# bitsauce/Carla-ppo

Measured on NVIDIA H100. Metric: VAE frames/sec @ batch 4096, higher is better.
Workload: dtype f32

## Files before the change

carla_ppo_b200/csrc/tapgemm.cuh:

```cuda
#pragma once
#include "common.cuh"

namespace cpb {

constexpr int kMaxTaps = 25;

struct Tap {
    int dy, dx;
    long long src_off;
    long long w_off;
};

struct TapClass {
    int ntaps;
    int py, px;
    int Ho, Wo;
    Tap taps[kMaxTaps];
};

struct TapGemmParams {
    const float* src;
    const float* wmat;
    const float* bias;
    const float* mask;
    float* dst;
    int batch;
    int Hs, Ws;
    int src_pitch;
    long long src_img;
    int sstride;
    int C;
    int N;
    int ldw;
    int Hd, Wd;
    int dstride;
    int dst_pitch;
    long long dst_img;
    int relu;
    int check;
    int nclass;
    int ybatch;
    long long w_ystride, bias_ystride, dst_ystride;
    int ksplit;
    float* kpartial;
    long long kpartial_stride;
    const float* wk_hi;
    const float* wk_lo;
    int quad;
    int quad_cb;
    int quad_lcb;
    int cluster;
    int debug;
    int passes;
    TapClass cls[4];
};

int32_t launch_tapgemm(const TapGemmParams& p, cudaStream_t stream);
constexpr int kMaxKSplit = 8;
int tapgemm_pick_ksplit(int rows, int N, int ybatch, int K);
int32_t launch_ksplit_reduce(const TapGemmParams& p, cudaStream_t stream);
int32_t tapgemm_init();

struct TcWeightJob {
    long long src_off;
    long long dst_hi, dst_lo;
    int mode;
    int k, cb, cs;
    int N, C;
    long long count;
    int round_nearest;
};
__host__ __device__ constexpr int tc_bn(int N) { return N % 64 == 0 ? 64 : 32; }
constexpr int kMaxTcWeightJobs = 12;
struct TcWeightTable {
    int njobs;
    long long total;
    TcWeightJob jobs[kMaxTcWeightJobs];
};
int32_t tc_tapgemm_init();
int tc_tapgemm_pick_ksplit(int K);
bool tc_tapgemm_supported(const TapGemmParams& p);
int32_t launch_tc_tapgemm(const TapGemmParams& p, cudaStream_t stream);
int32_t launch_tc_weights(const float* params, float* dst, const TcWeightTable& table, cudaStream_t stream);

}
```

carla_ppo_b200/csrc/tc_common.cuh:

```cuda
#pragma once
#include "common.cuh"

namespace cpb {
namespace tc {

constexpr int TBM = 128;
constexpr int TBK = 32;
constexpr int A_TILE_BYTES = TBM * TBK * 4;
constexpr int kMaxBN = 64;

__device__ __forceinline__ uint32_t smem_u32(const void* p) { return (uint32_t)__cvta_generic_to_shared(p); }

__host__ __device__ __forceinline__ uint32_t row_magic(int d) { return (uint32_t)((0x80000000ull + (uint32_t)d - 1) / (uint32_t)d); }
__device__ __forceinline__ int row_of(int rem, uint32_t magic) { return (int)__umulhi((uint32_t)rem << 1, magic); }

__device__ __forceinline__ void mbar_init(uint64_t* bar, uint32_t count) {
    asm volatile("mbarrier.init.shared::cta.b64 [%0], %1;" ::"r"(smem_u32(bar)), "r"(count));
}
__device__ __forceinline__ void mbar_wait(uint64_t* bar, uint32_t parity) {
    const uint32_t addr = smem_u32(bar);
    uint32_t ok = 0;
    for (uint32_t spin = 0; !ok; ++spin) {
        asm volatile(
            "{\n\t.reg .pred p;\n\t"
            "mbarrier.try_wait.parity.shared::cta.b64 p, [%1], %2;\n\t"
            "selp.u32 %0, 1, 0, p;\n\t}"
            : "=r"(ok)
            : "r"(addr), "r"(parity)
            : "memory");
        if (spin > (1u << 28)) __trap();
    }
}
__device__ __forceinline__ void mbar_arrive(uint64_t* bar) {
    asm volatile("{\n\t.reg .b64 st;\n\tmbarrier.arrive.shared::cta.b64 st, [%0];\n\t}" ::"r"(smem_u32(bar)) : "memory");
}
__device__ __forceinline__ void mbar_arrive_cluster(uint64_t* bar, uint32_t rank) {
    asm volatile(
        "{\n\t.reg .b32 ra;\n\t"
        "mapa.shared::cluster.u32 ra, %0, %1;\n\t"
        "mbarrier.arrive.release.cluster.shared::cluster.b64 _, [ra];\n\t}"
        ::"r"(smem_u32(bar)), "r"(rank) : "memory");
}
__device__ __forceinline__ void fence_async_smem() { asm volatile("fence.proxy.async.shared::cta;" ::: "memory"); }

__device__ __forceinline__ uint64_t make_desc(uint32_t smem_addr) {
    uint64_t d = 0;
    d |= (uint64_t)((smem_addr >> 4) & 0x3FFF);
    d |= (uint64_t)1 << 16;
    d |= (uint64_t)(1024 >> 4) << 32;
    d |= (uint64_t)1 << 62;
    return d;
}

__device__ __forceinline__ void wgmma_fence() { asm volatile("wgmma.fence.sync.aligned;" ::: "memory"); }
__device__ __forceinline__ void wgmma_commit() { asm volatile("wgmma.commit_group.sync.aligned;" ::: "memory"); }
template <int N>
__device__ __forceinline__ void wgmma_wait() { asm volatile("wgmma.wait_group.sync.aligned %0;" ::"n"(N) : "memory"); }
template <int R>
__device__ __forceinline__ void fence_regs(float* d) {
#pragma unroll
    for (int i = 0; i < R; ++i) asm volatile("" : "+f"(d[i])::"memory");
}

template <int N>
__device__ __forceinline__ void wgmma_tf32(float* d, uint64_t adesc, uint64_t bdesc, uint32_t scale_d);
template <>
__device__ __forceinline__ void wgmma_tf32<32>(float* d, uint64_t adesc, uint64_t bdesc, uint32_t scale_d) {
    asm volatile(
        "{\n\t.reg .pred p;\n\t"
        "setp.ne.b32 p, %18, 0;\n\t"
        "wgmma.mma_async.sync.aligned.m64n32k8.f32.tf32.tf32 {%0,%1,%2,%3,%4,%5,%6,%7,%8,%9,%10,%11,%12,%13,%14,%15}, %16, %17, p, 1, 1;\n\t}"
        : "+f"(d[0]), "+f"(d[1]), "+f"(d[2]), "+f"(d[3]), "+f"(d[4]), "+f"(d[5]), "+f"(d[6]), "+f"(d[7]), "+f"(d[8]), "+f"(d[9]), "+f"(d[10]), "+f"(d[11]), "+f"(d[12]), "+f"(d[13]), "+f"(d[14]), "+f"(d[15])
        : "l"(adesc), "l"(bdesc), "r"(scale_d));
}

template <>
__device__ __forceinline__ void wgmma_tf32<64>(float* d, uint64_t adesc, uint64_t bdesc, uint32_t scale_d) {
    asm volatile(
        "{\n\t.reg .pred p;\n\t"
        "setp.ne.b32 p, %34, 0;\n\t"
        "wgmma.mma_async.sync.aligned.m64n64k8.f32.tf32.tf32 {%0,%1,%2,%3,%4,%5,%6,%7,%8,%9,%10,%11,%12,%13,%14,%15,%16,%17,%18,%19,%20,%21,%22,%23,%24,%25,%26,%27,%28,%29,%30,%31}, %32, %33, p, 1, 1;\n\t}"
        : "+f"(d[0]), "+f"(d[1]), "+f"(d[2]), "+f"(d[3]), "+f"(d[4]), "+f"(d[5]), "+f"(d[6]), "+f"(d[7]), "+f"(d[8]), "+f"(d[9]), "+f"(d[10]), "+f"(d[11]), "+f"(d[12]), "+f"(d[13]), "+f"(d[14]), "+f"(d[15]), "+f"(d[16]), "+f"(d[17]), "+f"(d[18]), "+f"(d[19]), "+f"(d[20]), "+f"(d[21]), "+f"(d[22]), "+f"(d[23]), "+f"(d[24]), "+f"(d[25]), "+f"(d[26]), "+f"(d[27]), "+f"(d[28]), "+f"(d[29]), "+f"(d[30]), "+f"(d[31])
        : "l"(adesc), "l"(bdesc), "r"(scale_d));
}

template <int N>
__device__ __forceinline__ void wgmma_tf32_rs(float* d, const uint32_t* a, uint64_t bdesc, uint32_t scale_d);
template <>
__device__ __forceinline__ void wgmma_tf32_rs<32>(float* d, const uint32_t* a, uint64_t bdesc, uint32_t scale_d) {
    asm volatile(
        "{\n\t.reg .pred p;\n\t"
        "setp.ne.b32 p, %21, 0;\n\t"
        "wgmma.mma_async.sync.aligned.m64n32k8.f32.tf32.tf32 {%0,%1,%2,%3,%4,%5,%6,%7,%8,%9,%10,%11,%12,%13,%14,%15}, {%16,%17,%18,%19}, %20, p, 1, 1;\n\t}"
        : "+f"(d[0]), "+f"(d[1]), "+f"(d[2]), "+f"(d[3]), "+f"(d[4]), "+f"(d[5]), "+f"(d[6]), "+f"(d[7]), "+f"(d[8]), "+f"(d[9]), "+f"(d[10]), "+f"(d[11]), "+f"(d[12]), "+f"(d[13]), "+f"(d[14]), "+f"(d[15])
        : "r"(a[0]), "r"(a[1]), "r"(a[2]), "r"(a[3]), "l"(bdesc), "r"(scale_d));
}

template <>
__device__ __forceinline__ void wgmma_tf32_rs<64>(float* d, const uint32_t* a, uint64_t bdesc, uint32_t scale_d) {
    asm volatile(
        "{\n\t.reg .pred p;\n\t"
        "setp.ne.b32 p, %37, 0;\n\t"
        "wgmma.mma_async.sync.aligned.m64n64k8.f32.tf32.tf32 {%0,%1,%2,%3,%4,%5,%6,%7,%8,%9,%10,%11,%12,%13,%14,%15,%16,%17,%18,%19,%20,%21,%22,%23,%24,%25,%26,%27,%28,%29,%30,%31}, {%32,%33,%34,%35}, %36, p, 1, 1;\n\t}"
        : "+f"(d[0]), "+f"(d[1]), "+f"(d[2]), "+f"(d[3]), "+f"(d[4]), "+f"(d[5]), "+f"(d[6]), "+f"(d[7]), "+f"(d[8]), "+f"(d[9]), "+f"(d[10]), "+f"(d[11]), "+f"(d[12]), "+f"(d[13]), "+f"(d[14]), "+f"(d[15]), "+f"(d[16]), "+f"(d[17]), "+f"(d[18]), "+f"(d[19]), "+f"(d[20]), "+f"(d[21]), "+f"(d[22]), "+f"(d[23]), "+f"(d[24]), "+f"(d[25]), "+f"(d[26]), "+f"(d[27]), "+f"(d[28]), "+f"(d[29]), "+f"(d[30]), "+f"(d[31])
        : "r"(a[0]), "r"(a[1]), "r"(a[2]), "r"(a[3]), "l"(bdesc), "r"(scale_d));
}

__device__ __forceinline__ void split_tf32(float x, float& hi, float& lo) {
    hi = __uint_as_float(__float_as_uint(x) & 0xffffe000u);
    lo = x - hi;
}

__device__ __forceinline__ uint32_t round_tf32(float x) {
    uint32_t r;
    asm("cvt.rna.tf32.f32 %0, %1;" : "=r"(r) : "f"(x));
    return r;
}

}
}
```

carla_ppo_b200/csrc/tc_tapgemm.cu:

```cuda
#include "tapgemm.cuh"
#include "tc_common.cuh"

namespace cpb {

namespace {

using namespace tc;

template <int BN, int PASSES>
struct TcCfg {
    static constexpr int B_TILE_BYTES = BN * TBK * 4;
    static constexpr int B_IMAGES = PASSES == 3 ? 2 : 1;
    static constexpr int STAGE_BYTES = A_TILE_BYTES + B_IMAGES * B_TILE_BYTES;
    static constexpr int OUT_BYTES = TBM * BN * 4;
    static constexpr int STAGES = (224 * 1024 - OUT_BYTES) / STAGE_BYTES;
    static constexpr int SMEM_BYTES = STAGES * STAGE_BYTES + OUT_BYTES + 1024;
};
constexpr int CHUNK_KB = 4;

constexpr int kConsumerWarps = 8;
constexpr int kLoaderWarp0 = 8;
constexpr int kLoaderWarps = 4;
constexpr int kLoaderThreads = kLoaderWarps * 32;
constexpr int kEpilogueWarp0 = 12;
constexpr int kEpilogueWarps = 4;
constexpr int kEpilogueThreads = kEpilogueWarps * 32;
constexpr int kTcThreads = 512;
constexpr int kLaunchRegs = 128, kConsumerRegs = 168, kSideRegs = 80;
template <int R> __device__ __forceinline__ void reg_grow() { asm volatile("setmaxnreg.inc.sync.aligned.u32 %0;" ::"n"(R)); }
template <int R> __device__ __forceinline__ void reg_shrink() { asm volatile("setmaxnreg.dec.sync.aligned.u32 %0;" ::"n"(R)); }

int g_tc_cluster = 1;
int g_tc_clusters[2][2] = {{0, 0}, {0, 0}};

__device__ __forceinline__ uint32_t cluster_ctarank() { uint32_t r; asm volatile("mov.u32 %0, %%cluster_ctarank;" : "=r"(r)); return r; }
__device__ __forceinline__ uint32_t cluster_id_x() { uint32_t r; asm volatile("mov.u32 %0, %%clusterid.x;" : "=r"(r)); return r; }
__device__ __forceinline__ uint32_t cluster_count_x() { uint32_t r; asm volatile("mov.u32 %0, %%nclusterid.x;" : "=r"(r)); return r; }
__device__ __forceinline__ void cluster_sync_all() {
    asm volatile("barrier.cluster.arrive.release.aligned;" ::: "memory");
    asm volatile("barrier.cluster.wait.acquire.aligned;" ::: "memory");
}
__device__ __forceinline__ void mbar_expect_tx(uint64_t* bar, uint32_t bytes) {
    asm volatile("{\n\t.reg .b64 st;\n\tmbarrier.arrive.expect_tx.shared::cta.b64 st, [%0], %1;\n\t}" ::"r"(smem_u32(bar)), "r"(bytes) : "memory");
}
__device__ __forceinline__ void bulk_g2s(uint32_t dst, const void* src, uint32_t bytes, uint64_t* bar, uint16_t mask, bool multicast) {
    if (multicast)
        asm volatile("cp.async.bulk.shared::cluster.global.mbarrier::complete_tx::bytes.multicast::cluster [%0], [%1], %2, [%3], %4;"
                     ::"r"(dst), "l"(src), "r"(bytes), "r"(smem_u32(bar)), "h"(mask) : "memory");
    else
        asm volatile("cp.async.bulk.shared::cluster.global.mbarrier::complete_tx::bytes [%0], [%1], %2, [%3];"
                     ::"r"(dst), "l"(src), "r"(bytes), "r"(smem_u32(bar)) : "memory");
}

template <int BN, int PASSES, bool KSPLIT>
__global__ void __maxnreg__(kLaunchRegs)
tc_tapgemm_kernel(const __grid_constant__ TapGemmParams p, const int mgroups, const int total_w) {
    static_assert(PASSES == 3 || PASSES == 1, "3xTF32 or a single TF32 pass");
    using Cfg = TcCfg<BN, PASSES>;
    constexpr int STAGES = Cfg::STAGES;
    constexpr int B_TILE_BYTES = Cfg::B_TILE_BYTES;
    constexpr int STAGE_BYTES = Cfg::STAGE_BYTES;

    extern __shared__ uint8_t smem_raw[];
    __shared__ uint64_t full_bar[STAGES];
    __shared__ uint64_t empty_bar[STAGES];
    __shared__ uint64_t out_full;
    __shared__ uint64_t out_empty;

    const int tid = threadIdx.x;
    const int warp = __shfl_sync(0xffffffffu, tid >> 5, 0), lane = tid & 31;
    const int ntn = p.N / BN;
    const int CS = (int)p.cluster;
    const int rank = CS > 1 ? (int)cluster_ctarank() : 0;
    const int cl_id = CS > 1 ? (int)cluster_id_x() : (int)blockIdx.x;
    const int cl_n = CS > 1 ? (int)cluster_count_x() : (int)gridDim.x;
    const uint16_t cl_mask = (uint16_t)((1u << CS) - 1u);
    const uint32_t smem_base = (smem_u32(smem_raw) + 1023u) & ~1023u;
    const uint32_t out_base = smem_base + STAGES * STAGE_BYTES;

    if (tid == 0) {
#pragma unroll
        for (int s = 0; s < STAGES; ++s) { mbar_init(&full_bar[s], kLoaderThreads + 1); mbar_init(&empty_bar[s], (uint32_t)(kConsumerWarps * CS)); }
        mbar_init(&out_full, kConsumerWarps);
        mbar_init(&out_empty, kEpilogueWarps);
        asm volatile("fence.mbarrier_init.release.cluster;" ::: "memory");
    }
    __syncthreads();
    if (CS > 1) cluster_sync_all();

    auto st_z = [&](int st) { return st / (ntn * mgroups); };
    auto st_y = [&](int st) { return st % ntn; };
    auto st_m0 = [&](int st) { return (long long)(((st / ntn) % mgroups) * CS + rank) * TBM; };
    const int kb_per_tap = p.C / TBK;
    const int ksplit = KSPLIT ? p.ksplit : 1;
    auto split_kb = [&](int nkb, int ks) { return (int)((long long)nkb * ks / ksplit); };

    if (warp >= kEpilogueWarp0) {
        reg_shrink<kSideRegs>();
        constexpr int CPR = BN / 4;
        constexpr int RPP = kEpilogueThreads / CPR;
        constexpr int NR = TBM / RPP;
        constexpr uint32_t SKIP = 0xffffffffu;
        const int et = tid - kEpilogueWarp0 * 32;
        const int ec = et % CPR, er = et / CPR;
        const uint32_t o_src = out_base + (uint32_t)(er * (BN * 4) + ((ec ^ ((er & 3) << 1)) << 4));
        uint32_t phO = 0;
        for (int w = cl_id; w < total_w && !(p.debug & 16); w += cl_n) {
            const int st = KSPLIT ? w / ksplit : w, ks = KSPLIT ? w - st * ksplit : 0;
            const TapClass& cls = p.cls[st_z(st)];
            float* const dst = KSPLIT ? p.dst + (long long)ks * p.kpartial_stride : p.dst;
            const int Wo = cls.Wo, HoWo = cls.Ho * Wo;
            const uint32_t M = (uint32_t)p.batch * (uint32_t)HoWo;
            const uint32_t wo_magic = row_magic(Wo);
            const int col = st_y(st) * BN + ec * 4;
            int ch = col, qy = 0, qx = 0;
            if (p.quad) {
                const int c = col >> p.quad_lcb;
                ch = col & (p.quad_cb - 1);
                qy = c >> 1; qx = c & 1;
            }
            const uint32_t m0 = (uint32_t)st_m0(st) + (uint32_t)er;
            const int n0 = (int)(m0 / (uint32_t)HoWo);
            const int rem0 = (int)(m0 - (uint32_t)n0 * (uint32_t)HoWo);
            uint32_t m = m0;
            int n = n0, rem = rem0;
            auto next_off = [&]() {
                const int oy = row_of(rem, wo_magic);
                const int ox = rem - oy * Wo;
                const uint32_t img = (uint32_t)n * (uint32_t)p.dst_img;
                bool ok = m < M;
                uint32_t off;
                if (p.quad) {
                    const int y = oy * 2 + qy, x = ox * 2 + qx;
                    ok = ok && y < p.Hd && x < p.Wd;
                    off = img + (uint32_t)((y * p.Wd + x) * p.dst_pitch + ch);
                } else {
                    off = img + (uint32_t)(((oy * p.dstride + cls.py) * p.Wd + (ox * p.dstride + cls.px)) * p.dst_pitch + col);
                }
                m += RPP; rem += RPP;
                while (rem >= HoWo) { rem -= HoWo; ++n; }
                return ok ? off : SKIP;
            };
            uint32_t keep[NR / 8];
            if (p.mask) {
#pragma unroll 1
                for (int b = 0; b < NR / 8; ++b) {
                    uint32_t offs[8];
                    float4 mk[8];
#pragma unroll
                    for (int u = 0; u < 8; ++u) offs[u] = next_off();
#pragma unroll
                    for (int u = 0; u < 8; ++u)
                        mk[u] = offs[u] != SKIP ? __ldg(reinterpret_cast<const float4*>(p.mask + offs[u])) : make_float4(0.f, 0.f, 0.f, 0.f);
                    uint32_t bits = 0u;
#pragma unroll
                    for (int u = 0; u < 8; ++u)
                        bits |= ((mk[u].x > 0.f ? 1u : 0u) | (mk[u].y > 0.f ? 2u : 0u) | (mk[u].z > 0.f ? 4u : 0u) | (mk[u].w > 0.f ? 8u : 0u)) << (4 * u);
#pragma unroll
                    for (int q = 0; q < NR / 8 - 1; ++q) keep[q] = keep[q + 1];
                    keep[NR / 8 - 1] = bits;
                }
                m = m0; n = n0; rem = rem0;
            }
            float4 bias = make_float4(0.f, 0.f, 0.f, 0.f);
            if (p.bias) bias = __ldg(reinterpret_cast<const float4*>(p.bias + ch));

            mbar_wait(&out_full, phO);
            phO ^= 1u;
#pragma unroll 1
            for (int b = 0; b < NR / 8; ++b) {
                uint32_t offs[8];
                float4 sums[8];
#pragma unroll
                for (int u = 0; u < 8; ++u)
                    asm volatile("ld.shared.v4.f32 {%0, %1, %2, %3}, [%4];" : "=f"(sums[u].x), "=f"(sums[u].y), "=f"(sums[u].z), "=f"(sums[u].w)
                                 : "r"(o_src + (uint32_t)((8 * b + u) * RPP * BN * 4)));
#pragma unroll
                for (int u = 0; u < 8; ++u) offs[u] = next_off();
                const uint32_t bits = p.mask ? keep[0] : 0u;
#pragma unroll
                for (int q = 0; q < NR / 8 - 1; ++q) keep[q] = keep[q + 1];
#pragma unroll
                for (int u = 0; u < 8; ++u) {
                    if (offs[u] == SKIP) continue;
                    float4 o = sums[u];
                    if (p.bias) { o.x += bias.x; o.y += bias.y; o.z += bias.z; o.w += bias.w; }
                    if (p.relu) { o.x = fmaxf(o.x, 0.f); o.y = fmaxf(o.y, 0.f); o.z = fmaxf(o.z, 0.f); o.w = fmaxf(o.w, 0.f); }
                    if (p.mask) {
                        const uint32_t k = bits >> (4 * u);
                        o.x = (k & 1u) ? o.x : 0.f; o.y = (k & 2u) ? o.y : 0.f; o.z = (k & 4u) ? o.z : 0.f; o.w = (k & 8u) ? o.w : 0.f;
                    }
                    *reinterpret_cast<float4*>(dst + offs[u]) = o;
                }
            }
            __syncwarp();
            if (lane == 0) mbar_arrive(&out_empty);
        }
    } else if (warp >= kLoaderWarp0) {
        reg_shrink<kSideRegs>();
        const int tl = tid - kLoaderWarp0 * 32;
        const int a_chunk = tl & 7;
        const uint32_t a_soff0 = (uint32_t)((tl >> 6) * 1024 + ((tl >> 3) & 7) * 128 + ((a_chunk ^ ((tl >> 3) & 7)) << 4));
        constexpr int RPP = kLoaderThreads / 8;
        constexpr int RPT = TBM / RPP;

        int wA = cl_id, stA = 0, tapA = 0, cA = 0;
        int kbLeftA = 0;
        int ntapsA = 0;
        int offA = 0;
        uint32_t tapbitA = 1u;
        const TapClass* clsA = &p.cls[0];
        uint32_t a_base[RPT];
        uint32_t a_taps[RPT];
        auto setup_rows = [&]() {
            stA = KSPLIT ? wA / ksplit : wA;
            const int ksA = wA - stA * ksplit;
            clsA = &p.cls[st_z(stA)];
            ntapsA = clsA->ntaps;
            const int Wo = clsA->Wo, HoWo = clsA->Ho * Wo;
            const long long M = (long long)p.batch * HoWo;
            const uint32_t wo_magic = row_magic(Wo);
            long long m = st_m0(stA) + (tl >> 3);
            int n = (int)(m / HoWo);
            int rem = (int)(m - (long long)n * HoWo);
            int iy[RPT], ix[RPT];
#pragma unroll
            for (int i = 0; i < RPT; ++i) {
                const int oy = row_of(rem, wo_magic);
                const int ox = rem - oy * Wo;
                iy[i] = oy * p.sstride; ix[i] = ox * p.sstride;
                a_base[i] = (uint32_t)n * (uint32_t)p.src_img + (uint32_t)((iy[i] * p.Ws + ix[i]) * p.src_pitch + a_chunk * 4);
                a_taps[i] = m < M ? 0xffffffffu : 0u;
                m += RPP; rem += RPP;
                while (rem >= HoWo) { rem -= HoWo; ++n; }
            }
            if (p.check) {
                uint32_t in[RPT];
#pragma unroll
                for (int i = 0; i < RPT; ++i) in[i] = 0u;
                for (int t = 0; t < ntapsA; ++t) {
                    const int dy = clsA->taps[t].dy, dx = clsA->taps[t].dx;
#pragma unroll
                    for (int i = 0; i < RPT; ++i)
                        if ((unsigned)(iy[i] + dy) < (unsigned)p.Hs && (unsigned)(ix[i] + dx) < (unsigned)p.Ws) in[i] |= 1u << t;
                }
#pragma unroll
                for (int i = 0; i < RPT; ++i) a_taps[i] &= in[i];
            }
            if constexpr (KSPLIT) {
                const int nkb = ntapsA * kb_per_tap;
                const int kb0 = split_kb(nkb, ksA);
                kbLeftA = split_kb(nkb, ksA + 1) - kb0;
// ... 11 lines not shown
            const uint32_t dst = stage + a_soff0;
#pragma unroll
            for (int i = 0; i < RPT; ++i) {
                const bool v = (a_taps[i] & tapbitA) != 0u;
                const uint32_t off = v ? a_base[i] + (uint32_t)offA : 0u;
                const uint32_t bytes = (v && !(p.debug & 4)) ? 16u : 0u;
                if (p.debug & 2) continue;
                asm volatile("cp.async.cg.shared.global [%0], [%1], 16, %2;" ::"r"(dst + i * 2048), "l"(p.src + off), "r"(bytes) : "memory");
            }
            asm volatile("cp.async.mbarrier.arrive.noinc.shared::cta.b64 [%0];" ::"r"(smem_u32(full)) : "memory");
            cA += TBK; offA += TBK;
            if constexpr (KSPLIT) {
                if (--kbLeftA == 0) {
                    wA += cl_n;
                    if (wA < total_w) setup_rows();
                } else if (cA == p.C) {
                    cA = 0;
                    ++tapA;
                    offA = (int)clsA->taps[tapA].src_off;
                    tapbitA <<= 1;
                }
            } else if (cA == p.C) {
                cA = 0;
                if (++tapA == ntapsA) {
                    tapA = 0;
                    wA += cl_n;
                    if (wA < total_w) setup_rows();
                } else {
                    offA = (int)clsA->taps[tapA].src_off;
                    tapbitA <<= 1;
                }
            }
        };

        constexpr int B_BYTES = Cfg::B_IMAGES * B_TILE_BYTES;
        const uint32_t slice = (uint32_t)(B_BYTES / CS);
        auto issue_b = [&](uint32_t stage, uint64_t* full) {
            if (p.debug & 8) { mbar_arrive(full); return; }
            mbar_expect_tx(full, (uint32_t)B_BYTES);
            const float* wt = p.wk_hi + 2 * clsA->taps[tapA].w_off + ((long long)st_y(stA) * kb_per_tap + cA / TBK) * (2 * BN * TBK);
            bulk_g2s(stage + A_TILE_BYTES + (uint32_t)rank * slice, reinterpret_cast<const char*>(wt) + (size_t)rank * slice,
                     slice, full, cl_mask, CS > 1);
        };

        int sS = 0;
        uint32_t phS = 1;
        while (wA < total_w) {
            mbar_wait(&empty_bar[sS], phS);
            if (tl == 0) issue_b(smem_base + sS * STAGE_BYTES, &full_bar[sS]);
            issue_a(smem_base + sS * STAGE_BYTES, &full_bar[sS]);
            if (++sS == STAGES) { sS = 0; phS ^= 1u; }
        }
    } else {
        reg_grow<kConsumerRegs>();
        constexpr int HALF = BN / 2;
        const int wg = warp >> 2;
        float acc[HALF];
        float dm[HALF], dc[HALF];
#pragma unroll
        for (int i = 0; i < HALF; ++i) { acc[i] = 0.f; dm[i] = 0.f; dc[i] = 0.f; }

        auto release = [&](int s) {
            if (lane < CS) {
                if (CS > 1) mbar_arrive_cluster(&empty_bar[s], (uint32_t)lane);
                else mbar_arrive(&empty_bar[s]);
            }
        };

        const int r0 = wg * 64 + (warp & 3) * 16 + (lane >> 2);
        const uint32_t a_row = (uint32_t)((r0 >> 3) * 1024 + (r0 & 7) * 128 + (lane & 3) * 4);
        const uint32_t a_swz = (uint32_t)((r0 & 7) << 4);

        const uint32_t o_dst = (uint32_t)(r0 * (BN * 4) + ((r0 & 3) << 5) + (lane & 3) * 8);
        uint32_t phE = 1;
        auto hand_off = [&]() {
            mbar_wait(&out_empty, phE);
            phE ^= 1u;
#pragma unroll
            for (int j = 0; j < BN / 8; ++j)
#pragma unroll
                for (int h = 0; h < 2; ++h)
                    asm volatile("st.shared.v2.f32 [%0], {%1, %2};" ::"r"(out_base + (uint32_t)(h * 8 * BN * 4) + (o_dst ^ (uint32_t)(j << 5))),
                                 "f"(acc[4 * j + 2 * h]), "f"(acc[4 * j + 2 * h + 1]) : "memory");
            __syncwarp();
            if (lane == 0) mbar_arrive(&out_full);
        };

        int g = 0;
        for (int w = cl_id; w < total_w; w += cl_n) {
            const int st = KSPLIT ? w / ksplit : w, ks = KSPLIT ? w - st * ksplit : 0;
            const int nkb_tile = p.cls[st_z(st)].ntaps * kb_per_tap;
            const int nkb = KSPLIT ? split_kb(nkb_tile, ks + 1) - split_kb(nkb_tile, ks) : nkb_tile;
            for (int kb = 0; kb < nkb; ++kb, ++g) {
                const int s = g % STAGES;
                const uint32_t stage = smem_base + s * STAGE_BYTES;
                mbar_wait(&full_bar[s], (uint32_t)((g / STAGES) & 1));
                uint32_t ahi[TBK / 8][4], alo[TBK / 8][4];
#pragma unroll
                for (int ks = 0; ks < TBK / 8; ++ks)
#pragma unroll
                    for (int h = 0; h < 2; ++h)
#pragma unroll
                        for (int v = 0; v < 2; ++v) {
                            float x;
                            asm volatile("ld.shared.f32 %0, [%1];" : "=f"(x)
                                         : "r"(stage + a_row + v * 1024 + ((uint32_t)((2 * ks + h) << 4) ^ a_swz)));
                            if constexpr (PASSES == 3) {
                                float hi, lo;
                                split_tf32(x, hi, lo);
                                ahi[ks][2 * h + v] = __float_as_uint(hi);
                                alo[ks][2 * h + v] = __float_as_uint(lo);
                            } else {
                                ahi[ks][2 * h + v] = round_tf32(x);
                            }
                        }
#pragma unroll
                for (int ks = 0; ks < TBK / 8; ++ks)
#pragma unroll
                    for (int i = 0; i < 4; ++i) {
                        if constexpr (PASSES == 3) asm volatile("" : "+r"(ahi[ks][i]), "+r"(alo[ks][i]));
                        else asm volatile("" : "+r"(ahi[ks][i]));
                    }
                const uint64_t b_hi = make_desc(stage + A_TILE_BYTES);
                const uint64_t b_lo = make_desc(stage + A_TILE_BYTES + B_TILE_BYTES);
                wgmma_fence();
#pragma unroll
                for (int ks = 0; ks < TBK / 8; ++ks) {
                    const uint64_t adv = (uint64_t)(ks * 2);
                    const uint32_t keep = ((kb % CHUNK_KB) | ks) != 0 ? 1u : 0u;
                    wgmma_tf32_rs<BN>(dm, ahi[ks], b_hi + adv, keep);
                    if constexpr (PASSES == 3) {
                        wgmma_tf32_rs<BN>(dc, ahi[ks], b_lo + adv, keep);
                        wgmma_tf32_rs<BN>(dc, alo[ks], b_hi + adv, 1u);
                    }
                }
                wgmma_commit();
                wgmma_wait<0>();
                fence_regs<HALF>(dm);
                if constexpr (PASSES == 3) fence_regs<HALF>(dc);
                release(s);
                if (kb % CHUNK_KB == CHUNK_KB - 1 || kb == nkb - 1) {
#pragma unroll
                    for (int i = 0; i < HALF; ++i) {
                        acc[i] += dm[i];
                        if constexpr (PASSES == 3) acc[i] += dc[i];
                    }
                }
            }
            if (!(p.debug & 16)) hand_off();
#pragma unroll
            for (int i = 0; i < HALF; ++i) acc[i] = 0.f;
        }
    }
    __syncthreads();
    if (CS > 1) cluster_sync_all();
}

constexpr int tc_bn_slot(int BN) { return BN == 64 ? 1 : 0; }
constexpr int tc_passes_slot(int PASSES) { return PASSES == 1 ? 1 : 0; }

template <int BN, int PASSES, bool KSPLIT>
int32_t tc_launch_t(const TapGemmParams& p, int mgroups, int total_w, unsigned grid, cudaStream_t stream) {
    cudaLaunchConfig_t cfg;
    memset(&cfg, 0, sizeof(cfg));
    cfg.gridDim = dim3(grid);
    cfg.blockDim = dim3(kTcThreads);
    cfg.dynamicSmemBytes = TcCfg<BN, PASSES>::SMEM_BYTES;
    cfg.stream = stream;
    cudaLaunchAttribute attr;
    attr.id = cudaLaunchAttributeClusterDimension;
    attr.val.clusterDim.x = (unsigned)p.cluster; attr.val.clusterDim.y = 1; attr.val.clusterDim.z = 1;
    cfg.attrs = &attr; cfg.numAttrs = 1;
    CPB_CUDA(cudaLaunchKernelEx(&cfg, tc_tapgemm_kernel<BN, PASSES, KSPLIT>, p, mgroups, total_w));
    CPB_LAUNCHED();
    return CPB_OK;
}

template <int BN, int PASSES>
int32_t tc_launch(const TapGemmParams& p0, cudaStream_t stream) {
    long long max_m = 0;
    for (int c = 0; c < p0.nclass; ++c) {
        long long m = (long long)p0.batch * p0.cls[c].Ho * p0.cls[c].Wo;
        if (m > max_m) max_m = m;
    }
    if (max_m == 0) return CPB_OK;
    TapGemmParams p = p0;
    p.cluster = g_tc_cluster;
    const long long mtiles = (max_m + TBM - 1) / TBM;
    const long long mgroups = (mtiles + p.cluster - 1) / p.cluster;
    const long long total_w = mgroups * (p.N / BN) * p.nclass * p.ksplit;
    const int resident = g_tc_clusters[tc_passes_slot(PASSES)][tc_bn_slot(BN)];
    CPB_REQUIRE(total_w < (1ll << 30) && resident > 0, "tc_tapgemm: bad tile count");
    CPB_REQUIRE(tc_offsets_fit(p.batch, p.src_img) && tc_offsets_fit(p.batch, p.dst_img),
                "tc_tapgemm: tensors too large for 32-bit row offsets");
    auto al16 = [](const void* q) { return (reinterpret_cast<uintptr_t>(q) & 15u) == 0; };
    CPB_REQUIRE(al16(p.dst) && al16(p.mask) && al16(p.bias) && p.dst_pitch % 4 == 0 && p.dst_img % 4 == 0 &&
                    (p.ksplit == 1 || (al16(p.kpartial) && p.kpartial_stride % 4 == 0)),
                "tc_tapgemm: destination, mask and bias must be 16-byte aligned");
    for (int c = 0; c < p.nclass; ++c) CPB_REQUIRE(p.cls[c].ntaps <= 32, "tc_tapgemm: more than 32 taps");
    if (p.quad) {
        CPB_REQUIRE((p.quad_cb & (p.quad_cb - 1)) == 0, "tc_tapgemm: quad form needs a power-of-two channel count");
        p.quad_lcb = 0;
        while ((1 << p.quad_lcb) < p.quad_cb) ++p.quad_lcb;
    }
    const unsigned grid = (unsigned)((total_w < resident ? total_w : resident) * p.cluster);
    if (p.ksplit == 1) return tc_launch_t<BN, PASSES, false>(p, (int)mgroups, (int)total_w, grid, stream);
    if constexpr (PASSES == 1) {
        TapGemmParams q = p;
        q.dst = p.kpartial; q.bias = nullptr; q.mask = nullptr; q.relu = 0;
        CPB_TRY((tc_launch_t<BN, PASSES, true>(q, (int)mgroups, (int)total_w, grid, stream)));
        return launch_ksplit_reduce(p, stream);
    } else {
        CPB_REQUIRE(false, "tc_tapgemm: the k-split is built for the single TF32 pass only");
        return CPB_ERR_UNSUPPORTED;
    }
}

template <int BN, int PASSES>
int32_t tc_init_one() {
    using Cfg = TcCfg<BN, PASSES>;
    CPB_CUDA(cudaFuncSetAttribute(tc_tapgemm_kernel<BN, PASSES, false>, cudaFuncAttributeMaxDynamicSharedMemorySize, Cfg::SMEM_BYTES));
    if (g_tc_cluster > 1) CPB_CUDA(cudaFuncSetAttribute(tc_tapgemm_kernel<BN, PASSES, false>, cudaFuncAttributeNonPortableClusterSizeAllowed, 1));
    if constexpr (PASSES == 1) {
        CPB_CUDA(cudaFuncSetAttribute(tc_tapgemm_kernel<BN, PASSES, true>, cudaFuncAttributeMaxDynamicSharedMemorySize, Cfg::SMEM_BYTES));
        if (g_tc_cluster > 1) CPB_CUDA(cudaFuncSetAttribute(tc_tapgemm_kernel<BN, PASSES, true>, cudaFuncAttributeNonPortableClusterSizeAllowed, 1));
    }
    cudaLaunchConfig_t cfg;
    memset(&cfg, 0, sizeof(cfg));
    cfg.gridDim = dim3((unsigned)(g_tc_cluster * 1024));
    cfg.blockDim = dim3(kTcThreads);
    cfg.dynamicSmemBytes = Cfg::SMEM_BYTES;
    cudaLaunchAttribute attr;
    attr.id = cudaLaunchAttributeClusterDimension;
    attr.val.clusterDim.x = (unsigned)g_tc_cluster; attr.val.clusterDim.y = 1; attr.val.clusterDim.z = 1;
    cfg.attrs = &attr; cfg.numAttrs = 1;
    int n = 0;
    CPB_CUDA(cudaOccupancyMaxActiveClusters(&n, tc_tapgemm_kernel<BN, PASSES, false>, &cfg));
    CPB_REQUIRE(n > 0, "tc_tapgemm: no resident cluster of %d CTAs possible", g_tc_cluster);
    g_tc_clusters[tc_passes_slot(PASSES)][tc_bn_slot(BN)] = n;
    return CPB_OK;
}

__global__ void tc_weights_kernel(const float* __restrict__ params, float* __restrict__ dst, const __grid_constant__ TcWeightTable t) {
    long long idx = (long long)blockIdx.x * blockDim.x + threadIdx.x;
    if (idx >= t.total) return;
    int j = 0;
    while (j < t.njobs - 1 && idx >= t.jobs[j].count) { idx -= t.jobs[j].count; ++j; }
    const TcWeightJob& job = t.jobs[j];
    float x;
    int tap, n, c;
    if (job.mode == 0) {
        tap = 0; n = (int)(idx / job.C); c = (int)(idx % job.C);
        x = params[job.src_off + idx];
    } else if (job.mode == 3) {
        tap = 0; n = (int)(idx / job.C); c = (int)(idx % job.C);
        x = params[job.src_off + (long long)c * job.N + n];
    } else if (job.mode == 2) {
        const int w = (job.k + 1) / 2;
        const int cs = (int)(idx % job.cs);
        long long rest = idx / job.cs;
        const int ncol = (int)(rest % (4 * job.cb));
        rest /= (4 * job.cb);
        const int i = (int)(rest % w), jj = (int)(rest / w);
        const int cls = ncol / job.cb, cb = ncol - cls * job.cb;
        const int kh = (cls >> 1) + 2 * jj, kw = (cls & 1) + 2 * i;
        x = (kh < job.k && kw < job.k) ? params[job.src_off + (((long long)kh * job.k + kw) * job.cb + cb) * job.cs + cs] : 0.f;
        tap = jj * w + i; n = ncol; c = cs;
    } else {
        const int run = job.k * job.cb;
        const int cc = (int)(idx % run);
        const long long rest = idx / run;
        const int cs = (int)(rest % job.cs);
        const int kh = (int)(rest / job.cs);
        const int kw = cc / job.cb, cb = cc - kw * job.cb;
        x = params[job.src_off + (((long long)kh * job.k + kw) * job.cb + cb) * job.cs + cs];
        tap = kh; n = cs; c = cc;
    }
    const int BN = tc_bn(job.N);
    const int nn = n % BN, cc = c % TBK;
    const long long block = ((long long)tap * (job.N / BN) + n / BN) * (job.C / TBK) + c / TBK;
    const long long at = job.dst_hi + block * (2 * BN * TBK) + (nn >> 3) * 256 + (nn & 7) * 32 + ((((cc >> 2) ^ (nn & 7))) << 2) + (cc & 3);
    const float hi = job.round_nearest ? __uint_as_float(round_tf32(x)) : __uint_as_float(__float_as_uint(x) & 0xffffe000u);
    dst[at] = hi;
    if (!job.round_nearest) dst[at + BN * TBK] = x - hi;
}

}

int32_t tc_tapgemm_init() {
    const char* e = getenv("CPB_TC_CLUSTER");
    g_tc_cluster = e ? atoi(e) : 1;
    CPB_REQUIRE(g_tc_cluster == 1 || g_tc_cluster == 2 || g_tc_cluster == 4 || g_tc_cluster == 8, "CPB_TC_CLUSTER must be 1, 2, 4 or 8");
    CPB_TRY((tc_init_one<32, 3>()));
    CPB_TRY((tc_init_one<64, 3>()));
    CPB_TRY((tc_init_one<32, 1>()));
    CPB_TRY((tc_init_one<64, 1>()));
    return CPB_OK;
}

int tc_tapgemm_pick_ksplit(int K) {
    const int s = (int)cdiv(K / TBK, 320);
    return s < 1 ? 1 : (s > 4 ? 4 : s);
}

bool tc_tapgemm_supported(const TapGemmParams& p) {
    if (p.quad && (p.N != 4 * p.quad_cb || p.nclass != 1)) return false;
    if (p.ksplit < 1 || p.ksplit > kMaxKSplit) return false;
    if (p.ksplit > 1 && (p.nclass != 1 || p.quad || p.cls[0].Ho != 1 || p.cls[0].Wo != 1 || p.dst_pitch != p.N ||
                         p.kpartial == nullptr || p.cls[0].ntaps * (p.C / TBK) < p.ksplit))
        return false;
    return p.ybatch == 1 && p.C % TBK == 0 && p.N % 32 == 0 && p.N > 0 && p.wk_hi != nullptr && p.wk_lo != nullptr;
}

int32_t launch_tc_tapgemm(const TapGemmParams& p, cudaStream_t stream) {
    CPB_REQUIRE(tc_tapgemm_supported(p), "tc_tapgemm: unsupported problem (C=%d, N=%d)", p.C, p.N);
    CPB_REQUIRE(p.passes == 3 || p.passes == 1, "tc_tapgemm: passes must be 3 or 1, got %d", p.passes);
    if (p.passes == 1) return tc_bn(p.N) == 64 ? tc_launch<64, 1>(p, stream) : tc_launch<32, 1>(p, stream);
    return tc_bn(p.N) == 64 ? tc_launch<64, 3>(p, stream) : tc_launch<32, 3>(p, stream);
}

int32_t launch_tc_weights(const float* params, float* dst, const TcWeightTable& table, cudaStream_t stream) {
    if (table.total == 0) return CPB_OK;
    tc_weights_kernel<<<cdiv(table.total, 256), 256, 0, stream>>>(params, dst, table);
    CPB_LAUNCHED();
    return CPB_OK;
}

}
```

carla_ppo_b200/csrc/vae_api.cu:

```cuda
#include <algorithm>
#include <mutex>
#include <stdarg.h>

#include "elementwise.cuh"
#include "tapgemm.cuh"
#include "wgrad.cuh"

namespace cpb {

static thread_local char g_err[512] = "";
int64_t g_launches = 0;

void set_error(const char* fmt, ...) {
    va_list ap;
    va_start(ap, fmt);
    vsnprintf(g_err, sizeof(g_err), fmt, ap);
    va_end(ap);
}

bool g_profile_on = false;
namespace {
struct ProfRec { const char* label; cudaEvent_t a, b; };
constexpr int kMaxProfRecs = 4096;
ProfRec g_recs[kMaxProfRecs];
// ... 817 lines not shown
        int64_t widest = 0;
        for (int i = 0; i < p.nenc; ++i) widest = std::max<int64_t>(widest, p.enc[i]);
        for (int j = 0; j < p.ndec; ++j) widest = std::max<int64_t>(widest, p.dec[j]);
        p.ga = a.take<float>(b * widest);
        p.gb = a.take<float>(b * widest);
        p.gz = a.take<float>(b * zp);
        p.gheads = a.take<float>(2 * b * zp);
        int64_t o = 0;
        auto take = [&](int64_t n) { int64_t at = o; o += align_up(n, 64); return at; };
        for (int i = 1; i < p.nenc; ++i) p.tEnc[i] = take((int64_t)p.enc[i - 1] * p.enc[i]);
        p.tHeads = take(2LL * p.top() * zp);
        for (int j = 0; j < p.ndec; ++j) p.tDec[j] = take((j ? (int64_t)p.dec[j - 1] : zp) * p.dec[j]);
        p.tDec[p.ndec] = take((int64_t)p.last() * p.OUT);
        p.wT = a.take<float>(o);
        int widths[2 * kMlpMaxLayers + 3], nw = 0;
        widths[nw++] = p.IN;
        for (int i = 0; i < p.nenc; ++i) widths[nw++] = p.enc[i];
        widths[nw++] = p.zp;
        for (int j = 0; j < p.ndec; ++j) widths[nw++] = p.dec[j];
        widths[nw++] = p.OUT;
        int64_t best = 0;
        for (int k = 0; k + 1 < nw; ++k)
            best = std::max<int64_t>(best, (int64_t)wgrad_pick_splits(widths[k], widths[k + 1], b) * widths[k] * widths[k + 1]);
        p.partial = a.take<float>(best);
        p.colsum = a.take<float>(colsum_scratch_floats(b, p.OUT) + colsum_scratch_floats(b, (int)widest));
    }
    p.tc = g_math_mode == 2 && mlp_tc_batch_ok(b, p.IN);
    if (p.tc) {
        int64_t o = 0;
        auto take = [&](int64_t n) { int64_t at = o; o += align_up(n, 64); return at; };
        p.iE1 = take(2LL * p.enc[0] * p.IN);
        if (mode >= CPB_WS_FORWARD) p.iD3f = take(2LL * p.OUT * p.last());
        if (mode >= CPB_WS_TRAIN) p.iD3t = take(2LL * p.last() * p.OUT);
        p.wTc = a.take<float>(o);
        p.tcScratch = a.take<float>(mlp_tc_scratch_floats(p, mode));
    }
    p.bytes = a.off;
    return p;
}

static int32_t mlp_relayout_weights(const MlpPlan& pl, const MlpLayout& L, const float* params, bool encoder, bool decoder,
                                    bool backward, cudaStream_t s) {
    RelayoutTable t;
    memset(&t, 0, sizeof(t));
    add_z_padding(t, Latent{pl.B, pl.top(), pl.z, pl.zp, L.off, L.mean()}, true, pl.pHeads, pl.pHeadsB, true, L.off[L.dec(0)],
                  pl.dec[0], pl.pD1);
    CPB_TRY(launch_relayout(params, pl.wP, t, s));
    if (!pl.tc) return CPB_OK;
    TcWeightTable w;
    memset(&w, 0, sizeof(w));
    auto add = [&](int tensor, int64_t dst, int mode, int N, int C) {
        TcWeightJob& j = w.jobs[w.njobs++];
        j.src_off = L.off[tensor]; j.dst_hi = j.dst_lo = dst; j.mode = mode; j.N = N; j.C = C; j.round_nearest = 1;
        j.count = (long long)N * C; w.total += j.count;
    };
    const int out = L.dec(pl.ndec);
    if (encoder) add(L.enc(0), pl.iE1, 3, pl.enc[0], pl.IN);
    if (decoder) add(out, pl.iD3f, 3, pl.OUT, pl.last());
    if (backward) add(out, pl.iD3t, 0, pl.last(), pl.OUT);
    ProfScope prof("mlp.tc_weights", s);
    return launch_tc_weights(params, pl.wTc, w, s);
}

static int32_t mlp_dense(const char* label, const MlpPlan& pl, TapGemmParams p, const float* image, cudaStream_t s) {
    ProfScope prof(label, s);
    if (image == nullptr) return launch_tapgemm(p, s);
    p.wk_hi = p.wk_lo = image;
    p.passes = 1;
    p.ksplit = tc_tapgemm_pick_ksplit(p.C);
    if (p.ksplit > 1) { p.kpartial = pl.tcScratch; p.kpartial_stride = (long long)p.batch * p.N; }
    return launch_tc_tapgemm(p, s);
}

static int32_t run_tc_dense_wgrad(const char* label, const float* big, int I, const float* small, int J, int B, float* partial,
                                  float* out, bool transposed, cudaStream_t s) {
    ProfScope prof(label, s);
    WgradParams w;
    memset(&w, 0, sizeof(w));
    w.big = big; w.small = small; w.partial = partial;
    w.batch = B; w.Wb = 1; w.big_pitch = I; w.big_img = I; w.Ho = w.Wo = 1; w.sstride = 1;
    w.ntaps = 1; w.run = I; w.tap_off[0] = 0; w.I = I; w.J = J; w.passes = 1;
    w.splits = tc_wgrad_pick_splits(I, J, B);
    w.m_per_split = align_up(((long long)B + w.splits - 1) / w.splits, 32);
    CPB_TRY(launch_tc_wgrad(w, s));
    if (transposed) return launch_reduce_partials_t(partial, w.splits, I, J, out, s);
    return launch_reduce_partials(partial, w.splits, I, J, I, I, J, out, s);
}

static int32_t mlp_encoder(const MlpPlan& pl, const MlpLayout& L, const cpb_mlpvae_spec* c, const float* params, const void* source,
                           int32_t* flags, cudaStream_t s) {
    const float sscale = c->base.source_dtype == CPB_FRAME_U8 ? 1.f / 255.f : 1.f;
    CPB_TRY(launch_prep_flat(source, c->base.source_dtype, sscale, (long long)pl.B * pl.IN, pl.x, flags, 1, s));
    TapGemmParams p = dense_problem(pl.x, pl.B, pl.IN, params + L.off[L.enc(0)], pl.enc[0], params + L.off[L.enc(0) + 1],
                                    nullptr, pl.h[0], 1);
    CPB_TRY(mlp_dense("mlp.enc.fwd", pl, p, pl.tc ? pl.wTc + pl.iE1 : nullptr, s));
    for (int i = 1; i < pl.nenc; ++i) {
        p = dense_problem(pl.h[i - 1], pl.B, pl.enc[i - 1], params + L.off[L.enc(i)], pl.enc[i], params + L.off[L.enc(i) + 1],
                          nullptr, pl.h[i], 1);
        CPB_TRY(launch_tapgemm(p, s));
    }
    return launch_tapgemm(heads_fwd_problem(Latent{pl.B, pl.top(), pl.z, pl.zp, L.off, L.mean()}, params, pl.h[pl.nenc - 1],
                                            pl.wP + pl.pHeads, pl.wP + pl.pHeadsB, pl.heads), s);
}

static int32_t mlp_decoder(const MlpPlan& pl, const MlpLayout& L, const float* params, const float* zsrc, float* logits, cudaStream_t s) {
    const float* src = zsrc;
// ... 771 lines not shown
```

Before: 79750.

## Add BN=128 tensor-core tap-GEMM tile with shared-memory accumulation

Adds a 128-wide N tile for the TF32 wgmma tap-GEMM, using m64n128k8 instructions, whenever N is a multiple of 128 and no k-split applies. The wide tile raises A-tile reuse per loaded fragment. To fit within the register budget, it keeps running sums in the shared output buffer instead of a register accumulator array, and rebalances setmaxnreg across the consumer, loader and epilogue warps. The weight relayout and tile selection now depend on the k-split decision. Larger tiles cut the pipeline stage count and add shared-memory read-modify-write traffic, and some layers may get fewer CTAs.

```diff
diff --git a/carla_ppo_b200/csrc/tapgemm.cuh b/carla_ppo_b200/csrc/tapgemm.cuh
--- a/carla_ppo_b200/csrc/tapgemm.cuh
+++ b/carla_ppo_b200/csrc/tapgemm.cuh
@@ -69,8 +69,9 @@
     int N, C;
     long long count;
     int round_nearest;
+    int ksplit;
 };
-__host__ __device__ constexpr int tc_bn(int N) { return N % 64 == 0 ? 64 : 32; }
+__host__ __device__ constexpr int tc_bn(int N, bool ksplit) { return N % 128 == 0 && !ksplit ? 128 : (N % 64 == 0 ? 64 : 32); }
 constexpr int kMaxTcWeightJobs = 12;
 struct TcWeightTable {
     int njobs;
diff --git a/carla_ppo_b200/csrc/tc_common.cuh b/carla_ppo_b200/csrc/tc_common.cuh
--- a/carla_ppo_b200/csrc/tc_common.cuh
+++ b/carla_ppo_b200/csrc/tc_common.cuh
@@ -7,7 +7,7 @@
 constexpr int TBM = 128;
 constexpr int TBK = 32;
 constexpr int A_TILE_BYTES = TBM * TBK * 4;
-constexpr int kMaxBN = 64;
+constexpr int kMaxBN = 128;
 
 __device__ __forceinline__ uint32_t smem_u32(const void* p) { return (uint32_t)__cvta_generic_to_shared(p); }
 
@@ -106,6 +106,16 @@
         : "r"(a[0]), "r"(a[1]), "r"(a[2]), "r"(a[3]), "l"(bdesc), "r"(scale_d));
 }
 
+template <>
+__device__ __forceinline__ void wgmma_tf32_rs<128>(float* d, const uint32_t* a, uint64_t bdesc, uint32_t scale_d) {
+    asm volatile(
+        "{\n\t.reg .pred p;\n\t"
+        "setp.ne.b32 p, %69, 0;\n\t"
+        "wgmma.mma_async.sync.aligned.m64n128k8.f32.tf32.tf32 {%0,%1,%2,%3,%4,%5,%6,%7,%8,%9,%10,%11,%12,%13,%14,%15,%16,%17,%18,%19,%20,%21,%22,%23,%24,%25,%26,%27,%28,%29,%30,%31,%32,%33,%34,%35,%36,%37,%38,%39,%40,%41,%42,%43,%44,%45,%46,%47,%48,%49,%50,%51,%52,%53,%54,%55,%56,%57,%58,%59,%60,%61,%62,%63}, {%64,%65,%66,%67}, %68, p, 1, 1;\n\t}"
+        : "+f"(d[0]), "+f"(d[1]), "+f"(d[2]), "+f"(d[3]), "+f"(d[4]), "+f"(d[5]), "+f"(d[6]), "+f"(d[7]), "+f"(d[8]), "+f"(d[9]), "+f"(d[10]), "+f"(d[11]), "+f"(d[12]), "+f"(d[13]), "+f"(d[14]), "+f"(d[15]), "+f"(d[16]), "+f"(d[17]), "+f"(d[18]), "+f"(d[19]), "+f"(d[20]), "+f"(d[21]), "+f"(d[22]), "+f"(d[23]), "+f"(d[24]), "+f"(d[25]), "+f"(d[26]), "+f"(d[27]), "+f"(d[28]), "+f"(d[29]), "+f"(d[30]), "+f"(d[31]), "+f"(d[32]), "+f"(d[33]), "+f"(d[34]), "+f"(d[35]), "+f"(d[36]), "+f"(d[37]), "+f"(d[38]), "+f"(d[39]), "+f"(d[40]), "+f"(d[41]), "+f"(d[42]), "+f"(d[43]), "+f"(d[44]), "+f"(d[45]), "+f"(d[46]), "+f"(d[47]), "+f"(d[48]), "+f"(d[49]), "+f"(d[50]), "+f"(d[51]), "+f"(d[52]), "+f"(d[53]), "+f"(d[54]), "+f"(d[55]), "+f"(d[56]), "+f"(d[57]), "+f"(d[58]), "+f"(d[59]), "+f"(d[60]), "+f"(d[61]), "+f"(d[62]), "+f"(d[63])
+        : "r"(a[0]), "r"(a[1]), "r"(a[2]), "r"(a[3]), "l"(bdesc), "r"(scale_d));
+}
+
 __device__ __forceinline__ void split_tf32(float x, float& hi, float& lo) {
     hi = __uint_as_float(__float_as_uint(x) & 0xffffe000u);
     lo = x - hi;
diff --git a/carla_ppo_b200/csrc/tc_tapgemm.cu b/carla_ppo_b200/csrc/tc_tapgemm.cu
--- a/carla_ppo_b200/csrc/tc_tapgemm.cu
+++ b/carla_ppo_b200/csrc/tc_tapgemm.cu
@@ -15,6 +15,9 @@
     static constexpr int OUT_BYTES = TBM * BN * 4;
     static constexpr int STAGES = (224 * 1024 - OUT_BYTES) / STAGE_BYTES;
     static constexpr int SMEM_BYTES = STAGES * STAGE_BYTES + OUT_BYTES + 1024;
+    static constexpr bool WIDE = BN == 128 && PASSES == 3;
+    static constexpr int CONSUMER_REGS = WIDE ? 192 : 168, LOADER_REGS = WIDE ? 56 : 80, EPILOGUE_REGS = WIDE ? 72 : 80;
+    static_assert(256 * CONSUMER_REGS + 128 * (LOADER_REGS + EPILOGUE_REGS) <= 512 * 128, "register file of one CTA");
 };
 constexpr int CHUNK_KB = 4;
 
@@ -26,12 +29,12 @@
 constexpr int kEpilogueWarps = 4;
 constexpr int kEpilogueThreads = kEpilogueWarps * 32;
 constexpr int kTcThreads = 512;
-constexpr int kLaunchRegs = 128, kConsumerRegs = 168, kSideRegs = 80;
+constexpr int kLaunchRegs = 128;
 template <int R> __device__ __forceinline__ void reg_grow() { asm volatile("setmaxnreg.inc.sync.aligned.u32 %0;" ::"n"(R)); }
 template <int R> __device__ __forceinline__ void reg_shrink() { asm volatile("setmaxnreg.dec.sync.aligned.u32 %0;" ::"n"(R)); }
 
 int g_tc_cluster = 1;
-int g_tc_clusters[2][2] = {{0, 0}, {0, 0}};
+int g_tc_clusters[2][3] = {};
 
 __device__ __forceinline__ uint32_t cluster_ctarank() { uint32_t r; asm volatile("mov.u32 %0, %%cluster_ctarank;" : "=r"(r)); return r; }
 __device__ __forceinline__ uint32_t cluster_id_x() { uint32_t r; asm volatile("mov.u32 %0, %%clusterid.x;" : "=r"(r)); return r; }
@@ -96,7 +99,7 @@
     auto split_kb = [&](int nkb, int ks) { return (int)((long long)nkb * ks / ksplit); };
 
     if (warp >= kEpilogueWarp0) {
-        reg_shrink<kSideRegs>();
+        reg_shrink<Cfg::EPILOGUE_REGS>();
         constexpr int CPR = BN / 4;
         constexpr int RPP = kEpilogueThreads / CPR;
         constexpr int NR = TBM / RPP;
@@ -197,7 +200,7 @@
             if (lane == 0) mbar_arrive(&out_empty);
         }
     } else if (warp >= kLoaderWarp0) {
-        reg_shrink<kSideRegs>();
+        reg_shrink<Cfg::LOADER_REGS>();
         const int tl = tid - kLoaderWarp0 * 32;
         const int a_chunk = tl & 7;
         const uint32_t a_soff0 = (uint32_t)((tl >> 6) * 1024 + ((tl >> 3) & 7) * 128 + ((a_chunk ^ ((tl >> 3) & 7)) << 4));
@@ -315,13 +318,18 @@
             if (++sS == STAGES) { sS = 0; phS ^= 1u; }
         }
     } else {
-        reg_grow<kConsumerRegs>();
+        reg_grow<Cfg::CONSUMER_REGS>();
         constexpr int HALF = BN / 2;
+        constexpr bool SACC = BN == 128;
         const int wg = warp >> 2;
-        float acc[HALF];
+        float acc[SACC ? 1 : HALF];
         float dm[HALF], dc[HALF];
 #pragma unroll
-        for (int i = 0; i < HALF; ++i) { acc[i] = 0.f; dm[i] = 0.f; dc[i] = 0.f; }
+        for (int i = 0; i < HALF; ++i) { dm[i] = 0.f; dc[i] = 0.f; }
+        if constexpr (!SACC) {
+#pragma unroll
+            for (int i = 0; i < HALF; ++i) acc[i] = 0.f;
+        }
 
         auto release = [&](int s) {
             if (lane < CS) {
@@ -331,8 +339,7 @@
         };
 
         const int r0 = wg * 64 + (warp & 3) * 16 + (lane >> 2);
-        const uint32_t a_row = (uint32_t)((r0 >> 3) * 1024 + (r0 & 7) * 128 + (lane & 3) * 4);
-        const uint32_t a_swz = (uint32_t)((r0 & 7) << 4);
+        const uint32_t a_row = (uint32_t)((r0 >> 3) * 1024 + (r0 & 7) * 128 + ((r0 & 7) << 4) + (lane & 3) * 4);
 
         const uint32_t o_dst = (uint32_t)(r0 * (BN * 4) + ((r0 & 3) << 5) + (lane & 3) * 8);
         uint32_t phE = 1;
@@ -359,6 +366,8 @@
                 const uint32_t stage = smem_base + s * STAGE_BYTES;
                 mbar_wait(&full_bar[s], (uint32_t)((g / STAGES) & 1));
                 uint32_t ahi[TBK / 8][4], alo[TBK / 8][4];
+                uint32_t a_at = stage + a_row;
+                asm volatile("" : "+r"(a_at));
 #pragma unroll
                 for (int ks = 0; ks < TBK / 8; ++ks)
 #pragma unroll
@@ -367,7 +376,7 @@
                         for (int v = 0; v < 2; ++v) {
                             float x;
                             asm volatile("ld.shared.f32 %0, [%1];" : "=f"(x)
-                                         : "r"(stage + a_row + v * 1024 + ((uint32_t)((2 * ks + h) << 4) ^ a_swz)));
+                                         : "r"((a_at ^ (uint32_t)((2 * ks + h) << 4)) + (uint32_t)(v * 1024)));
                             if constexpr (PASSES == 3) {
                                 float hi, lo;
                                 split_tf32(x, hi, lo);
@@ -403,23 +412,66 @@
                 if constexpr (PASSES == 3) fence_regs<HALF>(dc);
                 release(s);
                 if (kb % CHUNK_KB == CHUNK_KB - 1 || kb == nkb - 1) {
-#pragma unroll
-                    for (int i = 0; i < HALF; ++i) {
-                        acc[i] += dm[i];
-                        if constexpr (PASSES == 3) acc[i] += dc[i];
+                    if constexpr (SACC) {
+                        const bool first = kb < CHUNK_KB;
+                        if (first && !(p.debug & 16)) {
+                            mbar_wait(&out_empty, phE);
+                            phE ^= 1u;
+                        }
+                        uint32_t ob = out_base + o_dst;
+                        asm volatile("" : "+r"(ob));
+#pragma unroll
+                        for (int j0 = 0; j0 < BN / 8; j0 += 4) {
+                            float sum[4][2][2];
+#pragma unroll
+                            for (int j = 0; j < 4; ++j)
+#pragma unroll
+                                for (int h = 0; h < 2; ++h) {
+                                    sum[j][h][0] = 0.f; sum[j][h][1] = 0.f;
+                                    if (!first)
+                                        asm volatile("ld.shared.v2.f32 {%0, %1}, [%2];" : "=f"(sum[j][h][0]), "=f"(sum[j][h][1])
+                                                     : "r"((ob ^ (uint32_t)((j0 + j) << 5)) + (uint32_t)(h * 8 * BN * 4)) : "memory");
+                                }
+#pragma unroll
+                            for (int j = 0; j < 4; ++j)
+#pragma unroll
+                                for (int h = 0; h < 2; ++h) {
+#pragma unroll
+                                    for (int c = 0; c < 2; ++c) {
+                                        sum[j][h][c] += dm[4 * (j0 + j) + 2 * h + c];
+                                        if constexpr (PASSES == 3) sum[j][h][c] += dc[4 * (j0 + j) + 2 * h + c];
+                                    }
+                                    asm volatile("st.shared.v2.f32 [%0], {%1, %2};"
+                                                 ::"r"((ob ^ (uint32_t)((j0 + j) << 5)) + (uint32_t)(h * 8 * BN * 4)),
+                                                 "f"(sum[j][h][0]), "f"(sum[j][h][1]) : "memory");
+                                }
+                        }
+                    } else {
+#pragma unroll
+                        for (int i = 0; i < HALF; ++i) {
+                            acc[i] += dm[i];
+                            if constexpr (PASSES == 3) acc[i] += dc[i];
+                        }
                     }
                 }
             }
-            if (!(p.debug & 16)) hand_off();
-#pragma unroll
-            for (int i = 0; i < HALF; ++i) acc[i] = 0.f;
+            if constexpr (SACC) {
+                if (!(p.debug & 16)) {
+                    __syncwarp();
+                    if (lane == 0) mbar_arrive(&out_full);
+                }
+            } else {
+                if (!(p.debug & 16)) hand_off();
+#pragma unroll
+                for (int i = 0; i < HALF; ++i) acc[i] = 0.f;
+            }
         }
     }
     __syncthreads();
     if (CS > 1) cluster_sync_all();
 }
 
-constexpr int tc_bn_slot(int BN) { return BN == 64 ? 1 : 0; }
+constexpr int tc_bn_slot(int BN) { return BN == 128 ? 2 : (BN == 64 ? 1 : 0); }
 constexpr int tc_passes_slot(int PASSES) { return PASSES == 1 ? 1 : 0; }
 
 template <int BN, int PASSES, bool KSPLIT>
@@ -468,13 +520,13 @@
     }
     const unsigned grid = (unsigned)((total_w < resident ? total_w : resident) * p.cluster);
     if (p.ksplit == 1) return tc_launch_t<BN, PASSES, false>(p, (int)mgroups, (int)total_w, grid, stream);
-    if constexpr (PASSES == 1) {
+    if constexpr (PASSES == 1 && BN <= 64) {
         TapGemmParams q = p;
         q.dst = p.kpartial; q.bias = nullptr; q.mask = nullptr; q.relu = 0;
         CPB_TRY((tc_launch_t<BN, PASSES, true>(q, (int)mgroups, (int)total_w, grid, stream)));
         return launch_ksplit_reduce(p, stream);
     } else {
-        CPB_REQUIRE(false, "tc_tapgemm: the k-split is built for the single TF32 pass only");
+        CPB_REQUIRE(false, "tc_tapgemm: the k-split is built for the single TF32 pass at BN <= 64 only");
         return CPB_ERR_UNSUPPORTED;
     }
 }
@@ -484,7 +536,7 @@
     using Cfg = TcCfg<BN, PASSES>;
     CPB_CUDA(cudaFuncSetAttribute(tc_tapgemm_kernel<BN, PASSES, false>, cudaFuncAttributeMaxDynamicSharedMemorySize, Cfg::SMEM_BYTES));
     if (g_tc_cluster > 1) CPB_CUDA(cudaFuncSetAttribute(tc_tapgemm_kernel<BN, PASSES, false>, cudaFuncAttributeNonPortableClusterSizeAllowed, 1));
-    if constexpr (PASSES == 1) {
+    if constexpr (PASSES == 1 && BN <= 64) {
         CPB_CUDA(cudaFuncSetAttribute(tc_tapgemm_kernel<BN, PASSES, true>, cudaFuncAttributeMaxDynamicSharedMemorySize, Cfg::SMEM_BYTES));
         if (g_tc_cluster > 1) CPB_CUDA(cudaFuncSetAttribute(tc_tapgemm_kernel<BN, PASSES, true>, cudaFuncAttributeNonPortableClusterSizeAllowed, 1));
     }
@@ -539,7 +591,7 @@
         x = params[job.src_off + (((long long)kh * job.k + kw) * job.cb + cb) * job.cs + cs];
         tap = kh; n = cs; c = cc;
     }
-    const int BN = tc_bn(job.N);
+    const int BN = tc_bn(job.N, job.ksplit != 0);
     const int nn = n % BN, cc = c % TBK;
     const long long block = ((long long)tap * (job.N / BN) + n / BN) * (job.C / TBK) + c / TBK;
     const long long at = job.dst_hi + block * (2 * BN * TBK) + (nn >> 3) * 256 + (nn & 7) * 32 + ((((cc >> 2) ^ (nn & 7))) << 2) + (cc & 3);
@@ -556,8 +608,10 @@
     CPB_REQUIRE(g_tc_cluster == 1 || g_tc_cluster == 2 || g_tc_cluster == 4 || g_tc_cluster == 8, "CPB_TC_CLUSTER must be 1, 2, 4 or 8");
     CPB_TRY((tc_init_one<32, 3>()));
     CPB_TRY((tc_init_one<64, 3>()));
+    CPB_TRY((tc_init_one<128, 3>()));
     CPB_TRY((tc_init_one<32, 1>()));
     CPB_TRY((tc_init_one<64, 1>()));
+    CPB_TRY((tc_init_one<128, 1>()));
     return CPB_OK;
 }
 
@@ -578,8 +632,9 @@
 int32_t launch_tc_tapgemm(const TapGemmParams& p, cudaStream_t stream) {
     CPB_REQUIRE(tc_tapgemm_supported(p), "tc_tapgemm: unsupported problem (C=%d, N=%d)", p.C, p.N);
     CPB_REQUIRE(p.passes == 3 || p.passes == 1, "tc_tapgemm: passes must be 3 or 1, got %d", p.passes);
-    if (p.passes == 1) return tc_bn(p.N) == 64 ? tc_launch<64, 1>(p, stream) : tc_launch<32, 1>(p, stream);
-    return tc_bn(p.N) == 64 ? tc_launch<64, 3>(p, stream) : tc_launch<32, 3>(p, stream);
+    const int bn = tc_bn(p.N, p.ksplit > 1);
+    if (p.passes == 1) return bn == 128 ? tc_launch<128, 1>(p, stream) : bn == 64 ? tc_launch<64, 1>(p, stream) : tc_launch<32, 1>(p, stream);
+    return bn == 128 ? tc_launch<128, 3>(p, stream) : bn == 64 ? tc_launch<64, 3>(p, stream) : tc_launch<32, 3>(p, stream);
 }
 
 int32_t launch_tc_weights(const float* params, float* dst, const TcWeightTable& table, cudaStream_t stream) {
diff --git a/carla_ppo_b200/csrc/vae_api.cu b/carla_ppo_b200/csrc/vae_api.cu
--- a/carla_ppo_b200/csrc/vae_api.cu
+++ b/carla_ppo_b200/csrc/vae_api.cu
@@ -893,6 +893,7 @@
     auto add = [&](int tensor, int64_t dst, int mode, int N, int C) {
         TcWeightJob& j = w.jobs[w.njobs++];
         j.src_off = L.off[tensor]; j.dst_hi = j.dst_lo = dst; j.mode = mode; j.N = N; j.C = C; j.round_nearest = 1;
+        j.ksplit = tc_tapgemm_pick_ksplit(C) > 1;
         j.count = (long long)N * C; w.total += j.count;
     };
     const int out = L.dec(pl.ndec);
```

Result: faster. 86060 (median of 6 runs) (+7.9%).
